# ban-m/jtk

Measured on AMD Instinct MI355X. Metric: chunks clustered/sec (whole node), 60x ONT 2kbp chunks, higher is better.
Workload: dtype f64

## Files before the change

### jtk_amd/csrc/polish_kernels.hip

```cpp
#include "device_common.h"

namespace {

__device__ __forceinline__ uint32_t edit_inserted(uint32_t row, uint32_t pos, uint32_t L) {
    if (row >= 4 && row < 8) return 1;
    if (row >= 8 && row < 11) {
        const uint32_t c = row - 7;
        return pos + c <= L ? c : L - pos;
    }
    return 0;
}

template <class Chunk>
__device__ __forceinline__ void select_edits_body(Chunk &&chunk, const ChunkMeta *chunks, ChunkState *state, const DevBufs &bufs,
                                                  const double *total_all, Edit *edits_all, uint32_t *new_len,
                                                  uint32_t ignore_edge, int final_pass) {
    extern __shared__ unsigned char s_best[];
    const uint32_t ci = chunk();
    ChunkState *st = &state[ci];
    if (st->status != 0 || !st->active) return;
    const ChunkMeta cm = chunks[ci];
    const uint32_t L = st->tmpl_len;
    if (final_pass) {
        if (threadIdx.x == 0) {
            st->active = 0;
            st->n_edits = 0;
        }
        return;
    }
    const double *total = total_all + cm.total_off;
    for (uint32_t p = threadIdx.x; p < L; p += 64) {
        uint32_t best = 0;
        double g = total[p * JTK_NUM_ROW];
        for (uint32_t row = 1; row < JTK_NUM_ROW; row++) {
            const double v = total[p * JTK_NUM_ROW + row];
            if (v > g) {
                g = v;
                best = row;
            }
        }
        s_best[p] = (unsigned char)(best | (g > JTK_POLISH_MIN_GAIN ? 0x80u : 0u));
    }
    __syncthreads();
    if (threadIdx.x != 0) return;
    const uint32_t round = st->rounds;
    const uint32_t inactive = 5 + (5 * round) % 21;
    Edit *edits = edits_all + cm.edit_off;
    uint32_t ne = 0, pos = ignore_edge, grow = 0;
    while (pos + ignore_edge < L) {
        const unsigned char b = s_best[pos];
        if ((b & 0x80u) && ne < cm.edit_cap) {
            const uint32_t row = b & 0x7fu;
            edits[ne].pos = pos;
            edits[ne].row = row;
            ne++;
            grow += edit_inserted(row, pos, L);
            pos += (row >= 11 ? row - 10 : 1) + inactive;
        } else {
            pos++;
        }
    }
    st->rounds = round + 1;
    st->n_edits = ne;
    if (ne == 0) {
        st->active = 0;
        return;
    }
    if (L + grow > cm.tmpl_cap) {
        st->status = JTK_ERR_CHUNK_FAILED;
        return;
    }
    const uint8_t *src = bufs.tmpl[st->buf] + cm.tmpl_off;
    uint8_t *dst = bufs.tmpl[JTK_NEXT_BUF(st->buf)] + cm.tmpl_off;
    uint32_t w = 0, e = 0, p = 0;
    while (p < L) {
        if (e < ne && edits[e].pos == p) {
            const uint32_t row = edits[e].row;
            e++;
            if (row < 4) {
                dst[w++] = (uint8_t)row;
                p++;
            } else if (row < 8) {
                dst[w++] = (uint8_t)(row - 4);
                dst[w++] = src[p++];
            } else if (row < 11) {
                const uint32_t c = row - 7;
                for (uint32_t q = 0; q < c && p + q < L; q++) dst[w++] = src[p + q];
                dst[w++] = src[p++];
            } else {
                p += row - 10;
            }
        } else {
            dst[w++] = src[p++];
        }
    }
    new_len[ci] = w;
}
__global__ __launch_bounds__(64) void select_edits_kernel(const RoundSegTable t, const RoundFirst f) {
    const uint32_t i = round_segment_of(f, blockIdx.x);
    const RoundSegment &g = t.seg[i];
    const uint32_t ci = blockIdx.x - f.first[i];
    select_edits_body([=] { return ci; }, g.chunks, g.state, g.bufs, g.total, g.edits, g.new_len, g.ignore_edge, g.final_pass);
}

#define RT_WAVES 4
__global__ __launch_bounds__(64 * RT_WAVES) void rethread_kernel(const RoundSegTable t, const RoundFirst f) {
    const uint32_t i = round_segment_of(f, blockIdx.x);
    const RoundSegment &g = t.seg[i];
    const uint32_t bid = blockIdx.x - f.first[i], n_reads = g.n_reads;
    const ReadMeta *reads = g.reads;
    const ChunkMeta *chunks = g.chunks;
    ChunkState *state = g.state;
    const DevBufs &bufs = g.bufs;
    const uint8_t *ey_all = g.ey;
    const Edit *edits_all = g.edits;
    const uint32_t lane = threadIdx.x & 63u;
    const uint32_t r = bid * RT_WAVES + (threadIdx.x >> 6);
    if (r >= n_reads) return;
    const ReadMeta rm = reads[r];
    ChunkState *st = &state[rm.chunk];
    if (st->status != 0 || !st->active || st->n_edits == 0) return;
    const ChunkMeta cm = chunks[rm.chunk];
    const uint32_t L = st->tmpl_len, ne = st->n_edits, b = st->buf, nb = JTK_NEXT_BUF(b);
    const Edit *edits = edits_all + cm.edit_off;
    const uint8_t *ops = bufs.ops[b] + rm.ops_off;
    uint8_t *out = bufs.ops[nb] + rm.ops_off;
    const uint32_t n_ops = bufs.ops_len[b][r];
    const uint8_t *tmpl = bufs.tmpl[nb] + cm.tmpl_off;
    const uint8_t *ey = ey_all + rm.ey_off;
    const unsigned long long below = (1ull << lane) - 1ull;
    uint32_t w0 = 0, ti0 = 0, ni0 = 0, nj0 = 0;
    uint32_t e_cur = 0;
    bool overflow = false;
    if (edits[0].pos == 0 && edits[0].row >= 4 && edits[0].row < 11) {
        const uint32_t k = edit_inserted(edits[0].row, 0, L);
        if (lane < k && lane < rm.ops_cap) out[lane] = JTK_OP_DEL;
        overflow = overflow || k > rm.ops_cap;
        w0 = k;
        ni0 = k;
    }
    for (uint32_t base = 0; base < n_ops; base += 64) {
        const uint32_t kk = base + lane;
        const bool has = kk < n_ops;
        const uint32_t op = has ? ops[kk] : (uint32_t)JTK_OP_INS;
        const bool cons = has && op != JTK_OP_INS;
        const unsigned long long mc = __ballot(cons);
        const uint32_t ti = ti0 + (uint32_t)__popcll(mc & below);
        while (e_cur < ne) {
            const Edit ed = edits[e_cur];
            const uint32_t last = ed.row >= 11 ? ed.pos + (ed.row - 10) - 1 : (ed.row >= 4 ? ed.pos - 1 : ed.pos);
            if ((ed.row >= 4 && ed.row < 11 && ed.pos == 0) || last < ti0)
                e_cur++;
            else
                break;
        }
        uint32_t first = has ? op : 4u;
        uint32_t k_del = 0;
        if (cons) {
            for (uint32_t e = e_cur; e < ne; e++) {
                const Edit ed = edits[e];
                if (ed.pos > ti + 1) break;
                if (ed.row >= 11) {
                    if (ed.pos <= ti && ti < ed.pos + (ed.row - 10)) first = op != JTK_OP_DEL ? (uint32_t)JTK_OP_INS : 4u;
                } else if (ed.row >= 4 && ed.pos == ti + 1) {
                    k_del = edit_inserted(ed.row, ed.pos, L);
                }
            }
        }
        const uint32_t c_out = (first != 4u ? 1u : 0u) + k_del;
        const uint32_t c_t = ((first <= JTK_OP_MISMATCH || first == JTK_OP_DEL) ? 1u : 0u) + k_del;
        const uint32_t c_r = (first <= JTK_OP_MISMATCH || first == JTK_OP_INS) ? 1u : 0u;
        const uint32_t packed = c_out | c_t << 10 | c_r << 20;
        uint32_t incl = packed;
#pragma unroll
        for (int o = 1; o < 64; o <<= 1) {
            const uint32_t u = __shfl_up(incl, o, 64);
            if ((int)lane >= o) incl += u;
        }
        const uint32_t excl = incl - packed, total = __shfl(incl, 63, 64);
        uint32_t w = w0 + (excl & 1023u);
        const uint32_t ni = ni0 + ((excl >> 10) & 1023u), nj = nj0 + (excl >> 20);
        if (first != 4u) {
            uint32_t o1 = first;
            if (first <= JTK_OP_MISMATCH) o1 = tmpl[ni] == (ey[nj + 1] & 3) ? JTK_OP_MATCH : JTK_OP_MISMATCH;
            if (w < rm.ops_cap) out[w] = (uint8_t)o1;
            w++;
        }
        for (uint32_t q = 0; q < k_del; q++)
            if (w + q < rm.ops_cap) out[w + q] = JTK_OP_DEL;
        w0 += total & 1023u;
        ni0 += (total >> 10) & 1023u;
        nj0 += total >> 20;
        ti0 += (uint32_t)__popcll(mc);
        overflow = overflow || w0 > rm.ops_cap;
    }
    if (lane == 0) {
        bufs.ops_len[nb][r] = overflow ? rm.ops_cap : w0;
        if (overflow) atomicMin(&st->status, (int)JTK_ERR_CHUNK_FAILED);
    }
}

__device__ __forceinline__ void commit_body(uint32_t n_chunks, ChunkState *state, const uint32_t *new_len, uint32_t *n_active,
                                            uint32_t *n_active_host) {
    uint32_t mine = 0;
    for (uint32_t ci = threadIdx.x; ci < n_chunks; ci += 256) {
        ChunkState *st = &state[ci];
        if (st->status != 0 || !st->active) continue;
        if (st->n_edits > 0) {
            st->buf = JTK_NEXT_BUF(st->buf);
            st->tmpl_len = new_len[ci];
            st->n_edits = 0;
        }
        mine++;
    }
    __shared__ uint32_t s_total;
    if (threadIdx.x == 0) s_total = 0;
    __syncthreads();
    if (mine) atomicAdd(&s_total, mine);
    __syncthreads();
    if (threadIdx.x == 0) {
        *n_active = s_total;
        if (n_active_host) __hip_atomic_store(n_active_host, s_total, __ATOMIC_RELAXED, __HIP_MEMORY_SCOPE_SYSTEM);
    }
}
__global__ __launch_bounds__(256) void commit_kernel(const RoundSegTable t, const RoundFirst f) {
    const RoundSegment &g = t.seg[round_segment_of(f, blockIdx.x)];
    commit_body(g.n_chunks, g.state, g.new_len, g.n_active + g.round, g.n_active_host ? g.n_active_host + g.round : nullptr);
}

__device__ __forceinline__ void reset_pass_body(const uint32_t bid, uint32_t n_chunks, ChunkState *state, const ChunkState *state0,
                                                uint32_t *n_active, uint32_t n_counters) {
    const uint32_t ci = bid * blockDim.x + threadIdx.x;
    if (ci < n_counters) n_active[ci] = 0;
    if (ci < n_chunks) state[ci] = state0[ci];
}
__global__ void reset_pass_kernel(const RoundSegTable t, const RoundFirst f) {
    const uint32_t i = round_segment_of(f, blockIdx.x);
    const RoundSegment &g = t.seg[i];
    reset_pass_body(blockIdx.x - f.first[i], g.n_chunks, g.state, g.state0, g.n_active, JTK_NACTIVE_SLOTS);
}

}

void launch_reset_pass(hipStream_t s, const RoundSegTable &t) {
    RoundFirst f;
    const uint32_t grid = round_prefix(t, f, [](const RoundSegment &g) {
        const uint32_t n = g.n_chunks > JTK_NACTIVE_SLOTS ? g.n_chunks : JTK_NACTIVE_SLOTS;
        return g.open ? (n + 127) / 128 : 0u;
    });
    if (grid) reset_pass_kernel<<<grid, 128, 0, s>>>(t, f);
}

void launch_polish_round(hipStream_t s, const RoundSegTable &t) {
    RoundFirst f;
    uint32_t max_tmpl = 0;
    for (uint32_t i = 0; i < t.n; i++)
        if (!t.seg[i].open && t.seg[i].max_tmpl > max_tmpl) max_tmpl = t.seg[i].max_tmpl;
    uint32_t grid = round_prefix(t, f, [](const RoundSegment &g) { return g.open ? 0u : g.n_chunks; });
    if (grid) select_edits_kernel<<<grid, 64, max_tmpl + 64, s>>>(t, f);
    grid = round_prefix(t, f, [](const RoundSegment &g) { return (g.open || g.final_pass || !g.n_chunks) ? 0u : (g.n_reads + RT_WAVES - 1) / RT_WAVES; });
    if (grid) rethread_kernel<<<grid, 64 * RT_WAVES, 0, s>>>(t, f);
    grid = round_prefix(t, f, [](const RoundSegment &g) { return (g.open || g.final_pass || !g.n_chunks) ? 0u : 1u; });
    if (grid) commit_kernel<<<grid, 256, 0, s>>>(t, f);
}
```

Before: 2833.

## Parallelize edit selection scan and template rebuild across the wavefront

The serial lane-0 scan over s_best, which picked edits and then rebuilt the template byte by byte, is replaced with a wave-wide ballot/ctz scan. Both the edit scan and the template copy now run across all 64 lanes: untouched runs are copied in parallel and edits are applied uniformly. The scan runs twice, once to count edits and growth and once to write the template, which adds redundant work and more control-flow complexity. Correctness depends on the uniform readfirstlane values and on the copy-run offsets matching the old semantics.

```diff
diff --git a/jtk_amd/csrc/polish_kernels.hip b/jtk_amd/csrc/polish_kernels.hip
--- a/jtk_amd/csrc/polish_kernels.hip
+++ b/jtk_amd/csrc/polish_kernels.hip
@@ -9,6 +9,32 @@
         return pos + c <= L ? c : L - pos;
     }
     return 0;
+}
+
+template <class OnEdit>
+__device__ __forceinline__ uint32_t scan_edits(const unsigned char *s_best, uint32_t L, uint32_t ignore_edge, uint32_t inactive,
+                                               uint32_t edit_cap, OnEdit &&on_edit) {
+    uint32_t ne = 0, pos = ignore_edge;
+    uint32_t base = 0xffffffffu;
+    uint64_t mask = 0;
+    while (pos + ignore_edge < L && ne < edit_cap) {
+        if ((pos & ~63u) != base) {
+            base = pos & ~63u;
+            const uint32_t p = base + threadIdx.x;
+            mask = __ballot(p + ignore_edge < L && (s_best[p] & 0x80u));
+        }
+        const uint64_t m = mask >> (pos & 63u);
+        if (m == 0) {
+            pos = base + 64;
+            continue;
+        }
+        pos += (uint32_t)__builtin_ctzll(m);
+        const uint32_t row = (uint32_t)__builtin_amdgcn_readfirstlane((int)(s_best[pos] & 0x7fu));
+        on_edit(pos, row);
+        ne++;
+        pos += (row >= 11 ? row - 10 : 1) + inactive;
+    }
+    return ne;
 }
 
 template <class Chunk>
@@ -20,7 +46,8 @@
     ChunkState *st = &state[ci];
     if (st->status != 0 || !st->active) return;
     const ChunkMeta cm = chunks[ci];
-    const uint32_t L = st->tmpl_len;
+    auto uni = [](uint32_t v) { return (uint32_t)__builtin_amdgcn_readfirstlane((int)v); };
+    const uint32_t L = uni(st->tmpl_len);
     if (final_pass) {
         if (threadIdx.x == 0) {
             st->active = 0;
@@ -28,8 +55,9 @@
         }
         return;
     }
+    const uint32_t lane = threadIdx.x;
     const double *total = total_all + cm.total_off;
-    for (uint32_t p = threadIdx.x; p < L; p += 64) {
+    for (uint32_t p = lane; p < L; p += 64) {
         uint32_t best = 0;
         double g = total[p * JTK_NUM_ROW];
         for (uint32_t row = 1; row < JTK_NUM_ROW; row++) {
@@ -42,59 +70,53 @@
         s_best[p] = (unsigned char)(best | (g > JTK_POLISH_MIN_GAIN ? 0x80u : 0u));
     }
     __syncthreads();
-    if (threadIdx.x != 0) return;
-    const uint32_t round = st->rounds;
+    const uint32_t round = uni(st->rounds), buf = uni(st->buf), edit_cap = uni(cm.edit_cap), tmpl_cap = uni(cm.tmpl_cap);
     const uint32_t inactive = 5 + (5 * round) % 21;
     Edit *edits = edits_all + cm.edit_off;
-    uint32_t ne = 0, pos = ignore_edge, grow = 0;
-    while (pos + ignore_edge < L) {
-        const unsigned char b = s_best[pos];
-        if ((b & 0x80u) && ne < cm.edit_cap) {
-            const uint32_t row = b & 0x7fu;
-            edits[ne].pos = pos;
-            edits[ne].row = row;
-            ne++;
-            grow += edit_inserted(row, pos, L);
-            pos += (row >= 11 ? row - 10 : 1) + inactive;
+    uint32_t grow = 0, k = 0;
+    const uint32_t ne = scan_edits(s_best, L, ignore_edge, inactive, edit_cap, [&](uint32_t pos, uint32_t row) {
+        if (lane == 0) {
+            edits[k].pos = pos;
+            edits[k].row = row;
+        }
+        k++;
+        grow += edit_inserted(row, pos, L);
+    });
+    __syncthreads();
+    if (lane == 0) {
+        st->rounds = round + 1;
+        st->n_edits = ne;
+        if (ne == 0) st->active = 0;
+        else if (L + grow > tmpl_cap) st->status = JTK_ERR_CHUNK_FAILED;
+    }
+    if (ne == 0 || L + grow > tmpl_cap) return;
+    const uint8_t *__restrict__ src = bufs.tmpl[buf] + cm.tmpl_off;
+    uint8_t *__restrict__ dst = bufs.tmpl[JTK_NEXT_BUF(buf)] + cm.tmpl_off;
+    uint32_t w = 0, p = 0;
+    auto copy_run = [&](uint32_t len) {
+        for (uint32_t q = lane; q < len; q += 64) dst[w + q] = src[p + q];
+        w += len;
+        p += len;
+    };
+    scan_edits(s_best, L, ignore_edge, inactive, edit_cap, [&](uint32_t pos, uint32_t row) {
+        copy_run(pos - p);
+        if (row < 4) {
+            if (lane == 0) dst[w] = (uint8_t)row;
+            w++;
+            p++;
+        } else if (row < 8) {
+            if (lane == 0) dst[w] = (uint8_t)(row - 4);
+            w++;
+        } else if (row < 11) {
+            const uint32_t c = edit_inserted(row, pos, L);
+            if (lane < c) dst[w + lane] = src[p + lane];
+            w += c;
         } else {
-            pos++;
-        }
-    }
-    st->rounds = round + 1;
-    st->n_edits = ne;
-    if (ne == 0) {
-        st->active = 0;
-        return;
-    }
-    if (L + grow > cm.tmpl_cap) {
-        st->status = JTK_ERR_CHUNK_FAILED;
-        return;
-    }
-    const uint8_t *src = bufs.tmpl[st->buf] + cm.tmpl_off;
-    uint8_t *dst = bufs.tmpl[JTK_NEXT_BUF(st->buf)] + cm.tmpl_off;
-    uint32_t w = 0, e = 0, p = 0;
-    while (p < L) {
-        if (e < ne && edits[e].pos == p) {
-            const uint32_t row = edits[e].row;
-            e++;
-            if (row < 4) {
-                dst[w++] = (uint8_t)row;
-                p++;
-            } else if (row < 8) {
-                dst[w++] = (uint8_t)(row - 4);
-                dst[w++] = src[p++];
-            } else if (row < 11) {
-                const uint32_t c = row - 7;
-                for (uint32_t q = 0; q < c && p + q < L; q++) dst[w++] = src[p + q];
-                dst[w++] = src[p++];
-            } else {
-                p += row - 10;
-            }
-        } else {
-            dst[w++] = src[p++];
-        }
-    }
-    new_len[ci] = w;
+            p += row - 10;
+        }
+    });
+    if (p < L) copy_run(L - p);
+    if (lane == 0) new_len[ci] = w;
 }
 __global__ __launch_bounds__(64) void select_edits_kernel(const RoundSegTable t, const RoundFirst f) {
     const uint32_t i = round_segment_of(f, blockIdx.x);
```

Result: no change. 2852, median of 2 (+0.6%).
